# tim-oster/voxel-rs

Measured on AMD Instinct MI355X. Metric: Mrays/sec (primary+shadow) at 1920x1080, depth-12 SVO; achieved HBM GB/s, higher is better.
Workload: dtype f32

## Files before the change

### profiles/timeline.py

```python
#!/usr/bin/env python3
import argparse
import json
import os
import sys
from pathlib import Path

os.environ["VX_TIMELINE"] = "1"
ROOT = Path(__file__).resolve().parent.parent
os.environ.setdefault("VX_LIB_DIR", str(ROOT / "voxel-rs_amd" / "lib" / "lib_tl"))
sys.path.insert(0, str(ROOT))
from _pkg import load_package

vra = load_package()
from voxel_rs_amd import hip, scenes


def main():
    ap = argparse.ArgumentParser()
    ap.add_argument("--format", default="esvo")
    ap.add_argument("--depth", type=int, default=12)
    ap.add_argument("--hot", default="1")
    ap.add_argument("--width", type=int, default=1920)
    ap.add_argument("--height", type=int, default=1080)
    args = ap.parse_args()
# ... 11 lines not shown
    svo.update(world)
    svo.set_frames_in_flight(1)
    u = scenes.bench_camera(args.depth, st["h_max"], W, H, shadow_distance=3.0e38, render_shadows=True)
    image = torch.zeros((H, W, 4), dtype=torch.float32, device="cuda")
    torch.cuda.synchronize()
    svo.profile_enable(True)
    for _ in range(6):
        svo.render_device(u, W, H, image.data_ptr())
    svo.sync()
    ms, launches = svo.profile_read()
    svo.profile_enable(False)
    raw = svo.timeline()
    r6 = raw[:, 6].copy()
    adv_only, push_only = ((r6 >> np.uint64(20)) & np.uint64(0xfffff)).astype(np.float64), ((r6 >> np.uint64(40)) & np.uint64(0xfffff)).astype(np.float64)
    raw[:, 6] = r6 & np.uint64(0xfffff)
    t = raw.astype(np.float64)
    t0 = t[:, 0].min()
    start, empty, leave = (t[:, 0] - t0) / 100.0, (t[:, 1] - t0) / 100.0, (t[:, 2] - t0) / 100.0
    q = lambda a: [round(float(np.percentile(a, p)), 1) for p in (0, 10, 50, 90, 99, 100)]
    r7 = t[:, 7].astype(np.uint64)
    wp, wt, wc = (r7 >> np.uint64(52)).astype(np.float64), ((r7 >> np.uint64(32)) & np.uint64(0xfffff)).astype(np.float64), (r7 & np.uint64(0xffffffff)).astype(np.float64)
    fit = [round(float(v), 1) for v in np.linalg.lstsq(np.stack([wp, wt], axis=1), wc, rcond=None)[0]] if wp.sum() > 0 else None
    print(json.dumps({"format": args.format, "hot_first": args.hot, "waves": int(len(t)), "percentiles": [0, 10, 50, 90, 99, 100],
                      "start_us": q(start), "queue_empty_us": q(empty[t[:, 1] > 0]), "exit_us": q(leave), "tail_us_per_wave": q((leave - empty)[t[:, 1] > 0]),
                      "subtiles_taken": q(t[:, 3].astype(np.uint64) & np.uint64(0xfffff)),
                      "service_phases_per_wave": q((t[:, 3].astype(np.uint64) >> np.uint64(20)) & np.uint64(0xfff)),
                      "us_in_service_phases_per_wave": q((t[:, 3].astype(np.uint64) >> np.uint64(32)).astype(np.float64) / 100.0), "kernel_us": round(float(leave.max()), 1),
                      "kernel_us_by_events_mean_of_launches": round(ms / max(launches, 1) * 1e3, 1),
                      "mean_wave_lifetime_us": round(float((leave - start).mean()), 1),
                      "clock_mhz": q(t[:, 4] / np.maximum(t[:, 2] - t[:, 0], 1.0) * 100.0),
                      "loop_share_of_wave_life": q(t[:, 5] / np.maximum(t[:, 4], 1.0)),
                      "loop_trips_per_wave": q(t[:, 6]),
                      "trips_by_tail_advance_only_push_only_merged": [round(float(adv_only.sum() / max(t[:, 6].sum(), 1.0)), 3), round(float(push_only.sum() / max(t[:, 6].sum(), 1.0)), 3),
                                                                      round(float(1.0 - (adv_only.sum() + push_only.sum()) / max(t[:, 6].sum(), 1.0)), 3)],
                      "cycles_per_trip_as_a_wave_sees_it": q(t[:, 5] / np.maximum(t[:, 6], 1.0)),
                      "cycles_per_trip_mean": round(float(t[:, 5].sum() / max(t[:, 6].sum(), 1.0)), 1),
                      "simd_cycles_per_trip_at_4_waves": round(float(t[:, 5].sum() / max(t[:, 6].sum(), 1.0)) / 4.0, 1),
                      "walk_phases_per_wave": q(wp), "walk_trips_per_wave": q(wt), "walk_cycles_per_wave": q(wc), "walk_fit_cycles_per_phase_and_per_trip": fit}))


if __name__ == "__main__":
    main()
```

### voxel-rs_amd/csrc/hip/comm.cpp

```cpp
#include <dlfcn.h>

#include <cstring>

#include "vx_context.hpp"

using vxrt::fail;
using vxrt::ProfiledLaunch;

namespace {

struct Rccl {
    void* lib = nullptr;
    decltype(&ncclGetUniqueId) GetUniqueId = nullptr;
    decltype(&ncclCommInitRank) CommInitRank = nullptr;
    decltype(&ncclCommDestroy) CommDestroy = nullptr;
    decltype(&ncclGroupStart) GroupStart = nullptr;
    decltype(&ncclGroupEnd) GroupEnd = nullptr;
    decltype(&ncclSend) Send = nullptr;
    decltype(&ncclRecv) Recv = nullptr;
    decltype(&ncclGetErrorString) GetErrorString = nullptr;
};
Rccl g_rccl;
std::string g_rccl_path;

// ... 102 lines not shown
int gather_tiles(vx_context* ctx, const void* tiles, uint64_t bytes_per_rank, void* gathered, int root, int* out_ticket, int only_slot);
}

int vx_gather_tiles(vx_context* ctx, const void* tiles, uint64_t bytes_per_rank, void* gathered, int root, int* out_ticket) {
    return gather_tiles(ctx, tiles, bytes_per_rank, gathered, root, out_ticket, -1);
}

namespace {
int gather_tiles(vx_context* ctx, const void* tiles, uint64_t bytes_per_rank, void* gathered, int root, int* out_ticket, int only_slot) {
    if (!ctx || !tiles || !bytes_per_rank || (bytes_per_rank & 3)) return fail(VX_ERR_INVALID_ARGUMENT, "gather_tiles: bad argument");
    VX_LOCK(ctx);
    if (!ctx->comm) return fail(VX_ERR_STATE, "gather_tiles: no communicator (vx_comm_init)");
    if (root < 0 || root >= ctx->comm_ranks) return fail(VX_ERR_INVALID_ARGUMENT, "gather_tiles: bad root");
    if (ctx->comm_rank == root && !gathered) return fail(VX_ERR_INVALID_ARGUMENT, "gather_tiles: the root needs a destination");
    HIP_TRY(hipSetDevice(ctx->device));
    if (only_slot >= 0 && only_slot < vx_context::kFrameStreams && ctx->frame_recorded[only_slot]) {
        HIP_TRY(hipStreamWaitEvent(ctx->comm_stream, ctx->frame_done[only_slot], 0));
    } else {
        if (ctx->render_recorded) HIP_TRY(hipStreamWaitEvent(ctx->comm_stream, ctx->render_done, 0));
        for (int i = 0; i < vx_context::kFrameStreams; ++i)
            if (ctx->frame_recorded[i]) HIP_TRY(hipStreamWaitEvent(ctx->comm_stream, ctx->frame_done[i], 0));
    }
    const size_t words = size_t(bytes_per_rank / 4);
    ProfiledLaunch ev{};
    if (ctx->profile) {
        if (!ctx->event_pool.empty()) {
            ev = ctx->event_pool.back();
            ctx->event_pool.pop_back();
        } else {
            HIP_TRY(hipEventCreate(&ev.start));
            HIP_TRY(hipEventCreate(&ev.stop));
        }
        HIP_TRY(hipEventRecord(ev.start, ctx->comm_stream));
    }
    auto exchange = [&]() -> int {
        if (ctx->comm_rank == root) {
// ... 95 lines not shown
```

### voxel-rs_amd/csrc/hip/kernels_render.hip

```cpp
#include <hip/hip_runtime.h>

#include "kernels.h"
#include "vx_device.hpp"
#include "vx_loop_gfx950.hpp"

#ifndef VX_ASM_LOOP
#define VX_ASM_LOOP 1
#endif
#ifndef VX_TIMELINE_BUILD
#define VX_TIMELINE_BUILD 0
#endif

using namespace vxd;
using namespace vxk;

namespace {


__device__ __forceinline__ uint32_t xcd_remap(uint32_t b, uint32_t n) {
    constexpr uint32_t X = 8;
    const uint32_t per = n / X, rem = n % X;
    const uint32_t xcd = b % X, slot = b / X;
    const uint32_t start = xcd * per + (xcd < rem ? xcd : rem);
    return start + slot;
// ... 157 lines not shown
    uint32_t out_index = 0;
    float primary_rd[3] = {0, 0, 0};
    float keep_color[4] = {0, 0, 0, 0}, keep_ds = 0.0f;
    float held_t = -1.0f;
    constexpr bool kDescendAlong = IMAGE && !HOT;
    vx_hit rec;
    uint32_t steps = 0;
    Counters ctr = {};
    uint32_t n_pixels = 0, lit = 0, shadow_rays = 0;
    uint32_t wave_steps = 0, services = 0, refills = 0, tail_wave_steps = 0, tail_iterations = 0;

    uint32_t cursor = 64, sub = 0;
    bool queue_empty = false;
    const unsigned long long t_start = a.timeline ? __builtin_amdgcn_s_memrealtime() : 0ull;
    unsigned long long t_empty = 0ull;
    uint32_t taken = 0;
    uint32_t in_service = 0, service_phases = 0;
    const unsigned long long c_start = a.timeline ? __builtin_amdgcn_s_memtime() : 0ull;
    unsigned long long loop_cycles = 0ull;
    uint32_t loop_trips = 0;
    unsigned long long loop_tails = 0ull;
    uint32_t my_queue = blockIdx.x & (kQueues - 1u);
    auto draw_raw = [&]() -> uint32_t {
        uint32_t raw = 0;
        if (lane == 0) raw = atomicAdd(a.work_counter + my_queue * kQueueStride, 1u);
        return raw;
    };
    auto region_ticket = [&](uint32_t k, uint32_t queue) -> uint32_t { return queue_subtile(k, queue, a.stripe, a.stripe_shift); };
    auto ticket_of = [&](uint32_t raw, uint32_t queue) -> uint32_t {
        return region_ticket(((gridDim.x + kQueues - 1u - queue) >> 3) + uint32_t(__builtin_amdgcn_readfirstlane(raw)), queue);
// ... 7 lines not shown
        for (uint32_t tried = 1; t >= a.total_subtiles && tried < kQueues; ++tried) {
            my_queue = (my_queue + 1u) & (kQueues - 1u);
            t = ticket_of(draw_raw(), my_queue);
        }
        return t;
    };
    if (blockIdx.x == 0 && lane < kQueues) a.next_counter[lane * kQueueStride] = 0u;
    uint32_t walk_cycles = 0, walk_trips = 0, walk_phases = 0;
    uint32_t my_chunk = 0, my_fill = 0;

    for (;;) {
        const uint32_t park_limit = a.service_min + uint32_t(__popcll(__ballot(state == kIdle || (FOREIGN == VX_SVO_CSVO && state == kForeign))));
        const uint32_t keep_going = park_limit >= 64u ? 0u : 64u - park_limit;
        unsigned long long trav = __ballot(tr.iter < uint32_t(kMaxSteps));
        const unsigned long long c_loop = a.timeline ? __builtin_amdgcn_s_memtime() : 0ull;
        constexpr bool kAsmLoop = VX_ASM_LOOP != 0 && IMAGE && (LV == kLdsLevels || LV == 16) && !HOT && !STATS;
        bool by_hand = false;
        if constexpr (kAsmLoop) {
            by_hand = __ballot((tr.flags & Trav<SVO>::kHasAdjacentLeaf) != 0 && tr.iter < uint32_t(kMaxSteps)) == 0;
            if (SVO == VX_SVO_IMAGE_WIDE && sc.wide_bytes >= (uint64_t(1) << 35)) by_hand = false;
        }
        if (kAsmLoop && by_hand) {
            if constexpr (kAsmLoop) {
                const uint32_t lds_base = uint32_t(reinterpret_cast<uintptr_t>(fast_st.at(0)));
                const uint32_t lds_slot0 = lds_base + fast_st.slot0;
                const uint32_t lds_aux0 = lds_base + 2u * FastStack::kPlane + uint32_t(int32_t(fast_st.slot0) >> 1);
                const uint32_t f_waiting = FOREIGN == VX_SVO_CSVO ? uint32_t(__popcll(__ballot(state == kForeign))) : 0u;
                const uint32_t f_min = FOREIGN == VX_SVO_CSVO ? 1u : 0xffffffffu;
                constexpr int kForeignKind = FOREIGN == VX_SVO_CSVO ? 1 : (FOREIGN == kForeignRerun ? 2 : 0);
                if (a.timeline) traverse_loop_gfx950<SVO, kForeignKind, true, LV>(tr, sc.records8, sc.wide, lds_slot0, lds_aux0, keep_going, f_waiting, f_min, loop_trips, &loop_tails);
// ... 324 lines not shown
                    }
                }
            }
        }
        VX_PART_END(4);
#undef VX_PART_BEGIN
#undef VX_PART_END
        if (a.timeline) { if (a.timeline_part == 0) in_service += uint32_t(__builtin_amdgcn_s_memrealtime() - t_service); ++service_phases; }
        if (__ballot(state != kIdle) == 0 && queue_empty) break;
    }

    if (a.timeline && lane == 0) {
        unsigned long long* row = a.timeline + size_t(blockIdx.x) * 8;
        row[0] = t_start; row[1] = t_empty; row[2] = __builtin_amdgcn_s_memrealtime();
        row[3] = taken | ((unsigned long long)(service_phases & 0xfffu) << 20) | ((unsigned long long)in_service << 32);
        row[4] = __builtin_amdgcn_s_memtime() - c_start; row[5] = loop_cycles;
        row[6] = (unsigned long long)(loop_trips & 0xfffffu) | ((loop_tails & 0xfffffull) << 20) | (((loop_tails >> 32) & 0xfffffull) << 40);
        row[7] = ((unsigned long long)(walk_phases & 0xfffu) << 52) | ((unsigned long long)(walk_trips & 0xfffffu) << 32) | walk_cycles;
    }
    if (FOREIGN == kForeignRerun || (FOREIGN == VX_SVO_CSVO && !HITS)) {
        const DevScene sc_bytes = vouched(make_scene(sa));
        Stack<64, false, false, int(FullStack::kStackBytes / (64u * 12u))> st2;
        st2.init(lane, &spill);
        const float to_light[3] = {-p.u.light_dir[0], -p.u.light_dir[1], -p.u.light_dir[2]};
        for (uint32_t c = my_chunk; c != 0;) {
            const uint32_t* chunk = todo.chunks + size_t(c - 1) * kRayChunkDwords;
            const uint32_t n = __builtin_amdgcn_readfirstlane(chunk[1]);
            c = __builtin_amdgcn_readfirstlane(chunk[0]);
            if (lane < n) {
                const uint4* w = reinterpret_cast<const uint4*>(chunk + kRayChunkHeader + lane * kRayRecordDwords);
                const uint4 w0 = w[0];
// ... 122 lines not shown
```

### voxel-rs_amd/csrc/hip/runtime.cpp

```cpp
#include <algorithm>
#include <chrono>
#include <cmath>
#include <cstdio>
#include <cstdlib>
#include <cstring>
#include <new>
#include <thread>

#include "vx_context.hpp"

using namespace vxd;
using namespace vxk;
using vxrt::check_ready;
using vxrt::fail;
using vxrt::g_last_error;
using vxrt::kWorldPad;
using vxrt::ProfiledLaunch;

namespace vxrt {
thread_local std::string g_last_error;
int fail(int code, const std::string& msg) {
    g_last_error = msg;
    return code;
}
// ... 9 lines not shown
    s.width = c->tex.width; s.height = c->tex.height; s.layers = c->tex.layers; s.levels = c->tex.levels;
    for (int l = 0; l < 16; ++l) s.level_offset[l] = c->tex.level_offset[l];
    return s;
}

int check_ready(vx_context* ctx) {
    if (!ctx) return fail(VX_ERR_INVALID_ARGUMENT, "null context");
    HIP_TRY(hipSetDevice(ctx->device));
    if (!ctx->committed) return fail(VX_ERR_STATE, "no SVO committed yet (call vx_commit / vx_commit_all first)");
    return VX_OK;
}

int mark_world_read(vx_context* ctx) {
    HIP_TRY(hipEventRecord(ctx->render_done, ctx->stream));
    ctx->render_recorded = true;
    return VX_OK;
}
}


namespace {
void wait_commit_idle(vx_context* ctx);
void stop_commit_worker(vx_context* ctx);
}

namespace {

constexpr size_t kImagePad = 64;
constexpr size_t kStagingSlack = 64;

// ... 217 lines not shown
            hs->width = p.width; hs->height = p.height; hs->tile_rank = p.tile_rank; hs->tile_count = p.tile_count;
        }
        a.stripe = 1;
        if (!a.order) a.stripe = ctx->queue_stripe > 0 ? uint32_t(ctx->queue_stripe) : 16u;
        if (a.stripe > a.total_subtiles) a.stripe = a.total_subtiles;
        if (a.stripe < 1u) a.stripe = 1u;
        a.stripe_shift = 0xffffffffu;
        for (uint32_t b = 0; b < 32u; ++b)
            if (a.stripe == (1u << b)) a.stripe_shift = b;
        int per_cu_used = per_cu;
        if (ctx->waves_per_cu_cap > 0 && ctx->waves_per_cu_cap < per_cu) per_cu_used = ctx->waves_per_cu_cap;
        else if (ctx->comm_ranks > 1 && ctx->comm_headroom > 0 && per_cu > ctx->comm_headroom + 4) per_cu_used = per_cu - ctx->comm_headroom;
        else if (p.tile_count > 1 || ctx->comm) per_cu_used = per_cu > 4 ? per_cu - 1 : per_cu;
        uint32_t waves = uint32_t(ctx->cu_count) * uint32_t(per_cu_used);
        if (waves > a.total_subtiles) waves = a.total_subtiles;
        if (waves > 8192) a.timeline = nullptr;
        ctx->timeline_waves = a.timeline ? waves : 0;
        PixelList todo = {nullptr, nullptr, 0};
        if (imaged && ctx->svo_type == VX_SVO_CSVO) {
            uint32_t*& ring = slot >= 0 ? ctx->d_frame_todo[slot] : ctx->d_main_todo;
            size_t& have = slot >= 0 ? ctx->frame_todo_chunks[slot] : ctx->main_todo_chunks;
            const bool ray_list = !HITS;
            const size_t need = ray_list ? (size_t(p.n_local_tiles) * kTile * kTile / kRayChunkRecords + waves + 1) * (kRayChunkDwords / kChunkDwords)
                                         : size_t(p.n_local_tiles) * kTile * kTile / 63 + waves + 1;
            if (have < need) {
                if (ring) {
                    HIP_TRY(hipStreamSynchronize(stream));
                    (void)hipFree(ring);
                    ring = nullptr;
                    have = 0;
                }
// ... 6 lines not shown
            todo.next_chunk = ring;
            todo.chunks = ring + 32;
            todo.mask = uint32_t((ray_list ? have / (kRayChunkDwords / kChunkDwords) : have) - 1);
        }
        void* kargs[] = {const_cast<SceneArgs*>(&sc), const_cast<RenderParams*>(&p), &a, &out, &hits, &counters, &todo};
        HIP_TRY(hipLaunchKernel(fn, dim3(waves), dim3(64), kargs, wave_lds, stream));
        tickets += 1u;
        order_after = hs;
        order_subtiles = a.total_subtiles;
    }
    HIP_TRY(hipGetLastError());
    if (ctx->profile) {
        HIP_TRY(hipEventRecord(ev.stop, stream));
        ctx->launches.push_back(ev);
    }
    if (slot >= 0) {
        HIP_TRY(hipEventRecord(ctx->frame_done[slot], stream));
        ctx->frame_recorded[slot] = true;
    } else {
        HIP_TRY(hipEventRecord(ctx->render_done, stream));
        ctx->render_recorded = true;
    }
    if (order_after) {
        vx_context::HotState* hs = order_after;
        const uint32_t g = hs->frames % 3;
        {
            HIP_TRY(hipStreamWaitEvent(ctx->order_stream, slot >= 0 ? ctx->frame_done[slot] : ctx->render_done, 0));
            HIP_TRY(vxk::launch_order(ctx->order_stream, hs->cost[g], hs->tag, order_subtiles, hs->order[g]));
            HIP_TRY(hipEventRecord(hs->order_done[g], ctx->order_stream));
        }
        hs->frames += 1;
    }
    ctx->last_frame_slot = slot;
    return VX_OK;
}

int apply_pending_waits(vx_context* ctx, hipStream_t stream) {
    if (ctx->pending_wait) HIP_TRY(hipStreamWaitEvent(stream, ctx->pending_wait, 0));
    if (ctx->pending_gather) HIP_TRY(hipStreamWaitEvent(stream, ctx->pending_gather, 0));
    ctx->pending_wait = nullptr;
    ctx->pending_gather = nullptr;
// ... 223 lines not shown
    {
        if (const char* e = std::getenv("VX_RENDER_KERNEL")) c->kernel_version = std::atoi(e) == 1 ? 1 : 2;
        if (const char* e = std::getenv("VX_FRAMES_IN_FLIGHT")) c->frames_in_flight = std::atoi(e);
        if (c->frames_in_flight < 1) c->frames_in_flight = 1;
        if (c->frames_in_flight > vx_context::kFrameStreams) c->frames_in_flight = vx_context::kFrameStreams;
        if (const char* e = std::getenv("VX_TRAVERSAL_IMAGE")) c->image_enabled = std::atoi(e) != 0;
        if (const char* e = std::getenv("VX_FOREIGN_RERUN")) c->foreign_rerun = std::atoi(e) != 0 ? 1 : 0;
        if (const char* e = std::getenv("VX_HOT_LEVELS")) c->hot_levels = std::atoi(e) != 0;
        if (const char* e = std::getenv("VX_IMAGE_CAP_BYTES")) c->image_cap_bytes = size_t(std::strtoull(e, nullptr, 10));
        if (const char* e = std::getenv("VX_IMAGE_FIRST_BYTES")) c->image_first_bytes = std::max<size_t>(4096, size_t(std::strtoull(e, nullptr, 10)));
        int wide_image = 0;
        if (const char* e = std::getenv("VX_WIDE_IMAGE")) wide_image = std::atoi(e);
        c->image = vximg::WorldImage(svo_type, wide_image ? vximg::kOct64Wide : vximg::kOct64, wide_image == 2 ? (uint64_t(5) << 30) / 4 : 0);
        if (const char* e = std::getenv("VX_COMM_HEADROOM")) c->comm_headroom = std::max(0, std::atoi(e));
        if (const char* e = std::getenv("VX_SERVICE_MIN")) c->service_min = uint32_t(std::atoi(e));
        c->tile_numbering = svo_type == VX_SVO_ESVO ? 2 : 1;
        if (const char* e = std::getenv("VX_TILE_NUMBERING")) c->tile_numbering = std::atoi(e);
        if (vxk::timeline_build()) {
            if (const char* e = std::getenv("VX_HOT_FIRST")) c->hot_first = std::atoi(e) != 0;
            if (const char* e = std::getenv("VX_TIMELINE"))
                if (std::atoi(e) != 0) CREATE_TRY(hipMalloc(reinterpret_cast<void**>(&c->d_timeline), 8192 * 8 * sizeof(unsigned long long)));
            if (const char* e = std::getenv("VX_TIMELINE_PART")) c->timeline_part = uint32_t(std::atoi(e));
            if (const char* e = std::getenv("VX_WAVES_PER_CU")) c->waves_per_cu_cap = std::atoi(e);
            if (const char* e = std::getenv("VX_REFILL_MIN")) c->refill_min = uint32_t(std::atoi(e));
            if (const char* e = std::getenv("VX_QUEUE_STRIPE")) c->queue_stripe = std::atoi(e);
            if (const char* e = std::getenv("VX_TILE_STRIP")) c->tile_strip = std::atoi(e);
        }
        if (c->refill_min < 1) c->refill_min = 1;
        if (c->refill_min > 64) c->refill_min = 64;
        if (c->service_min < 1) c->service_min = 1;
        if (c->service_min > 64) c->service_min = 64;
    }
    const vx_material zero_mat = {0, 0, -1, -1, -1, -1, -1, -1};
    CREATE_TRY(hipMalloc(reinterpret_cast<void**>(&c->d_materials), sizeof zero_mat));
    CREATE_TRY(hipMemcpy(c->d_materials, &zero_mat, sizeof zero_mat, hipMemcpyHostToDevice));
    c->n_materials = 1;
// ... 270 lines not shown
                drop_image();
            }
        }
    } else if (ctx->image_enabled && ctx->kernel_version != 1) {
        drop_image();
    }
    if (image_ok) {
        const uint8_t* src = reinterpret_cast<const uint8_t*>(ctx->image.frame().data());
        if (whole_image) {
            up.push_back(Upload{ctx->d_image, src, ctx->image.frame_bytes()});
        } else {
            for (const vximg::Range& r : ctx->image.dirty_bytes()) up.push_back(Upload{ctx->d_image + r.start, src + r.start, r.length});
        }
    }

    auto wait_for_frames = [&]() -> int {
        if (ctx->render_recorded) HIP_TRY(hipStreamWaitEvent(ctx->upload_stream, ctx->render_done, 0));
        for (int i = 0; i < vx_context::kFrameStreams; ++i)
            if (ctx->frame_recorded[i]) HIP_TRY(hipStreamWaitEvent(ctx->upload_stream, ctx->frame_done[i], 0));
        return VX_OK;
    };
    uint64_t total = 0;
    for (const Upload& u : up) total += u.bytes;
    int rc = VX_OK;
    if (total <= kDeltaLimit) {
        rc = upload_packed(ctx, up, wait_for_frames);
    } else {
        rc = wait_for_frames();
        if (rc == VX_OK) rc = upload_big(ctx, up);
    }
    if (rc != VX_OK) {
        const std::string why = g_last_error;
        drop_image();
        ctx->image_ok = false;
        g_last_error = why;
        return rc;
// ... 178 lines not shown
    if (ps.busy) HIP_TRY(hipEventSynchronize(ps.copied));
    if (ps.cap < bytes) {
        if (ps.dev) (void)hipFree(ps.dev);
        if (ps.host) (void)hipHostFree(ps.host);
        ps.dev = ps.host = nullptr;
        ps.cap = 0;
        HIP_TRY(hipMalloc(&ps.dev, bytes));
        HIP_TRY(hipHostMalloc(&ps.host, bytes, hipHostMallocDefault));
        ps.cap = bytes;
    }
    if (!ps.copied) HIP_TRY(hipEventCreateWithFlags(&ps.copied, hipEventDisableTiming));
    if (!ctx->copy_stream) HIP_TRY(hipStreamCreateWithFlags(&ctx->copy_stream, hipStreamNonBlocking));
    const int slot = ctx->frames_in_flight > 1 ? int(ctx->frame_index++ % unsigned(ctx->frames_in_flight)) : -1;
    if (int rc = apply_pending_waits(ctx, slot >= 0 ? ctx->frame_stream[slot] : ctx->stream)) return rc;
    if (int rc = launch_render(ctx, p, static_cast<float*>(ps.dev), nullptr, nullptr, slot)) return rc;
    HIP_TRY(hipStreamWaitEvent(ctx->copy_stream, slot >= 0 ? ctx->frame_done[slot] : ctx->render_done, 0));
    HIP_TRY(hipMemcpyAsync(ps.host, ps.dev, bytes, hipMemcpyDeviceToHost, ctx->copy_stream));
    HIP_TRY(hipEventRecord(ps.copied, ctx->copy_stream));
    ps.bytes = bytes;
    ps.busy = true;
    *out_slot = k;
    return VX_OK;
}

int vx_present_wait(vx_context* ctx, int slot, const void** pixels, size_t* bytes) {
    if (!ctx || slot < 0 || slot >= vx_context::kPresentSlots || !pixels) return fail(VX_ERR_INVALID_ARGUMENT, "present_wait: bad argument");
    VX_LOCK(ctx);
    vx_context::PresentSlot& ps = ctx->present[slot];
    if (!ps.busy) return fail(VX_ERR_STATE, "present_wait: nothing was begun on this slot");
    HIP_TRY(hipSetDevice(ctx->device));
// ... 122 lines not shown
    return VX_OK;
}

int vx_wait_event(vx_context* ctx, void* hip_event) {
    if (!ctx) return fail(VX_ERR_INVALID_ARGUMENT, "null context");
    VX_LOCK(ctx);
    ctx->pending_wait = static_cast<hipEvent_t>(hip_event);
    return VX_OK;
}

int vx_stream_wait_render(vx_context* ctx, void* stream) {
    if (!ctx) return fail(VX_ERR_INVALID_ARGUMENT, "null context");
    VX_LOCK(ctx);
    HIP_TRY(hipSetDevice(ctx->device));
    const int slot = ctx->last_frame_slot;
    if (slot >= 0) {
        if (ctx->frame_recorded[slot]) HIP_TRY(hipStreamWaitEvent(static_cast<hipStream_t>(stream), ctx->frame_done[slot], 0));
    } else if (ctx->render_recorded) {
        HIP_TRY(hipStreamWaitEvent(static_cast<hipStream_t>(stream), ctx->render_done, 0));
    }
    return VX_OK;
}

int vx_assemble_tiles(vx_context* ctx, const float* tiles, uint64_t stride_floats, uint32_t tile_count, uint32_t width, uint32_t height,
                      float* out_rgba32f) {
    if (!ctx) return fail(VX_ERR_INVALID_ARGUMENT, "null context");
    for (int i = 0; i < vx_context::kFrameStreams; ++i)
        if (ctx->frame_recorded[i]) HIP_TRY(hipStreamWaitEvent(ctx->stream, ctx->frame_done[i], 0));
    return vx_assemble_tiles_on(ctx, tiles, stride_floats, tile_count, width, height, out_rgba32f, ctx->stream);
}

int vx_assemble_tiles_on(vx_context* ctx, const float* tiles, uint64_t stride_floats, uint32_t tile_count, uint32_t width, uint32_t height,
                         float* out_rgba32f, void* stream) {
    if (stride_floats & 3) return fail(VX_ERR_INVALID_ARGUMENT, "assemble_tiles: the stride between the ranks' lists must be whole pixels (a multiple of 4 floats)");
    return vx_assemble_tiles_format(ctx, tiles, stride_floats / 4, tile_count, width, height, out_rgba32f, VX_FORMAT_RGBA32F, stream);
}

int vx_assemble_tiles_format(vx_context* ctx, const void* tiles, uint64_t stride_pixels, uint32_t tile_count, uint32_t width, uint32_t height, void* out,
                             int format, void* stream) {
    if (!ctx || !tiles || !out || !tile_count || !width || !height || (format != VX_FORMAT_RGBA32F && format != VX_FORMAT_RGBA8))
        return fail(VX_ERR_INVALID_ARGUMENT, "assemble_tiles: bad argument");
    const uintptr_t align = format == VX_FORMAT_RGBA32F ? 15u : 3u;
    if ((reinterpret_cast<uintptr_t>(tiles) & align) || (reinterpret_cast<uintptr_t>(out) & align))
// ... 87 lines not shown
        }
        if (!ctx->h_probe) HIP_TRY(hipHostMalloc(reinterpret_cast<void**>(&ctx->h_probe), 2 * sizeof(unsigned long long), hipHostMallocDefault));
        ctx->h_probe[0] = ctx->h_probe[1] = 0ull;
        HIP_TRY(vxk::launch_clock_probe(ctx->probe_stream, microseconds * 100u, ctx->h_probe));
    }
    HIP_TRY(hipStreamSynchronize(ctx->probe_stream));
    if (ctx->h_probe[1] == 0ull) return fail(VX_ERR_HIP, "clock_probe: the probe did not report");
    *shader_mhz = double(ctx->h_probe[0]) / double(ctx->h_probe[1]) * 100.0;
    return VX_OK;
}

uint32_t vx_timeline_read(vx_context* ctx, uint64_t* out, uint32_t capacity_waves) {
    if (!ctx || !ctx->d_timeline || !out) return 0;
    VX_LOCK(ctx);
    if (hipSetDevice(ctx->device) != hipSuccess || drain_streams(ctx) != VX_OK) return 0;
    const uint32_t n = ctx->timeline_waves < capacity_waves ? ctx->timeline_waves : capacity_waves;
    if (n && hipMemcpy(out, ctx->d_timeline, size_t(n) * 8 * sizeof(uint64_t), hipMemcpyDeviceToHost) != hipSuccess) return 0;
    return n;
}

int vx_image_info(const vx_context* ctx, uint64_t out[4]) {
    if (!ctx || !out) return fail(VX_ERR_INVALID_ARGUMENT, "image_info: null argument");
    VX_LOCK(const_cast<vx_context*>(ctx));
    out[0] = ctx->image_ok ? (ctx->pub.layout == vximg::kOct64Wide ? 2u : 1u) : 0u;
    out[1] = ctx->image_ok ? ctx->pub.frame_bytes : 0u;
    out[2] = ctx->image_ok ? ctx->pub.origin_bytes : 0u;
    out[3] = ctx->image_ok ? ctx->pub.chunks : 0u;
    return VX_OK;
}

// ... 28 lines not shown
```

### voxel-rs_amd/csrc/hip/vx_context.hpp

```cpp
#pragma once

#include <hip/hip_runtime_api.h>
#include <rccl/rccl.h>

#include <condition_variable>
#include <mutex>
#include <string>
#include <thread>
#include <unordered_map>
#include <vector>

#include "kernels.h"
#include "traversal_image.hpp"
#include "voxel_hip.h"
#include "vx_args.hpp"

namespace vxrt {

extern thread_local std::string g_last_error;
int fail(int code, const std::string& msg);

#define HIP_TRY(call)                                                                                              \
    do {                                                                                                           \
        hipError_t e_ = (call);                                                                                    \
// ... 3 lines not shown

struct ProfiledLaunch {
    hipEvent_t start, stop;
};

}

struct vx_context;
namespace vxrt {
void comm_release(vx_context* c);

constexpr size_t kWorldPad = 16;
vxd::SceneArgs scene_on_bytes(const vx_context* c);
int check_ready(vx_context* ctx);
int mark_world_read(vx_context* ctx);
}

struct vx_context {
    int svo_type = 0;
    int device = 0;
    size_t capacity = 0;
    uint8_t* staging = nullptr;
    uint8_t* d_world = nullptr;
    hipStream_t stream = nullptr;
    hipStream_t upload_stream = nullptr;
    hipEvent_t upload_done = nullptr, render_done = nullptr;
    bool committed = false, render_recorded = false;
    static constexpr int kFrameStreams = 8;
    hipStream_t frame_stream[kFrameStreams] = {};
    hipEvent_t frame_done[kFrameStreams] = {};
    bool frame_recorded[kFrameStreams] = {};
    uint32_t* d_frame_counter[kFrameStreams] = {};
    uint32_t frame_tickets[kFrameStreams] = {};
    uint32_t* d_frame_todo[kFrameStreams] = {};
    size_t frame_todo_chunks[kFrameStreams] = {};
    uint32_t* d_main_todo = nullptr;
    size_t main_todo_chunks = 0;
    uint32_t main_tickets = 0;
    struct HotState {
        uint32_t* cost[3] = {nullptr, nullptr, nullptr};
        uint32_t* order[3] = {nullptr, nullptr, nullptr};
        hipEvent_t order_done[3] = {nullptr, nullptr, nullptr};
        size_t subtiles = 0;
        uint32_t tag = 0;
        uint32_t frames = 0;
        uint32_t width = 0, height = 0, tile_rank = 0, tile_count = 0;
// ... 17 lines not shown
    float* d_frame = nullptr;  size_t d_frame_bytes = 0;
    vx_hit* d_hits = nullptr;  size_t d_hits_bytes = 0;
    vx_picker_task* d_tasks = nullptr;  vx_picker_result* d_results = nullptr;  uint32_t picker_cap = 0;
    static constexpr uint32_t kPickerDirect = 2048;
    vx_picker_task* h_pick_tasks = nullptr;  vx_picker_result* h_pick_results = nullptr;
    vx_picker_task* d_pick_tasks = nullptr;  vx_picker_result* d_pick_results = nullptr;
    vx_result* d_trace_result = nullptr;  vx_frame* d_trace_frames = nullptr;  uint32_t* d_trace_count = nullptr;  uint32_t trace_cap = 0;
    unsigned long long* d_counters = nullptr;

    uint32_t* d_work_counter = nullptr;
    unsigned long long* d_excursions = nullptr;
    bool count_excursions = false;
    unsigned long long* d_timeline = nullptr;
    uint32_t timeline_waves = 0;
    uint32_t timeline_part = 0;
    vximg::WorldImage image;
    uint8_t* d_image = nullptr;
    size_t d_image_capacity = 0;
    uint8_t* d_origin = nullptr;
    size_t d_origin_capacity = 0;
    size_t image_cap_bytes = 0;
    size_t image_first_bytes = size_t(32) << 20;
    struct DeltaSlot { uint8_t* host = nullptr; uint8_t* dev = nullptr; size_t cap = 0; hipEvent_t done = nullptr; bool used = false; };
    static constexpr int kDeltaSlots = 3;
    DeltaSlot delta[kDeltaSlots];
    unsigned delta_next = 0;
    bool hot_levels = false;
    int foreign_rerun = -1;
    bool big = false;
    bool image_enabled = true;
    bool image_ok = false;
    int kernel_version = 2;
    uint32_t refill_min = 64, service_min = 64;
    int tile_strip = 8;
    int tile_numbering = 1;
    int queue_stripe = 0;
    std::vector<vx_material> host_materials;
    std::vector<uint8_t> opaque_layer;
    uint64_t opaque_blocks = 0;
    int waves_per_cu_cap = 0;
    int comm_headroom = 4;
    int cu_count = 256;
    std::unordered_map<const void*, int> persistent_blocks;

    struct TileTable { uint32_t tiles_x = 0, tiles_y = 0; uint32_t* d_order = nullptr; uint32_t* d_inverse = nullptr; };
    std::vector<TileTable> tile_tables;
    struct LaunchTable { uint32_t tiles_x = 0, tiles_y = 0, rank = 0, count = 0, numbering = 0, strip = 0; uint2* d_table = nullptr; uint32_t* d_number = nullptr; };
    std::vector<LaunchTable> launch_tables;

    ncclComm_t comm = nullptr;
    int comm_ranks = 0, comm_rank = 0;
    hipStream_t comm_stream = nullptr;
    static constexpr int kGatherEvents = 16;
    hipEvent_t gather_done[kGatherEvents] = {};
    unsigned gather_index = 0;
// ... 32 lines not shown
```

Measured before the change: 14000.

## Record render-done events lazily and cap waves for tile-list renders

Render launches now mark frames dirty instead of recording a completion event every launch. The event is recorded only when a consumer (gather, copy, upload, assemble) needs to wait on it, which trims per-frame host API calls. For sharded tile-list renders, the persistent wave count is capped to about three subtiles per wave (at least one wave per CU), so tiny launches carry less wave-launch overhead. Timeline instrumentation also gains multi-launch ring storage and a start-to-first-trip timestamp, plus new profiling scripts.

```diff
diff --git a/profiles/round7/ab_summary.py b/profiles/round7/ab_summary.py
--- /dev/null
+++ b/profiles/round7/ab_summary.py
@@ -0,0 +1,57 @@
+#!/usr/bin/env python3
+import glob
+import json
+import statistics
+import sys
+
+d = sys.argv[1]
+
+
+def lines(arm, mode):
+    out = []
+    for f in sorted(glob.glob(f"{d}/{arm}_{mode}_*.json")):
+        try:
+            out.append(json.loads(open(f).read()))
+        except ValueError:
+            pass
+    return out
+
+
+def fit_a(sm):
+    xs, ys = [1 / 2, 1 / 4, 1 / 8], [sm[n]["share_ms_mean"] for n in ("2", "4", "8")]
+    mx, my = sum(xs) / 3, sum(ys) / 3
+    b = sum((x - mx) * (y - my) for x, y in zip(xs, ys)) / sum((x - mx) ** 2 for x in xs)
+    return my - b * mx
+
+
+FIGURES = [("plain", "ms_per_step (plain run, one block of 50)", lambda j: j["ms_per_step"], True),
+           ("full", "ms_per_step burst (--full, median of 25 blocks)", lambda j: j["burst"]["ms_per_step"], True),
+           ("full", "ms_per_step sustained (--full, 3 s)", lambda j: j["sustained"]["ms_per_step"], True),
+           ("full", "scale_model share_ms_mean N=2", lambda j: j["scale_model"]["2"]["share_ms_mean"], True),
+           ("full", "scale_model share_ms_mean N=4", lambda j: j["scale_model"]["4"]["share_ms_mean"], True),
+           ("full", "scale_model share_ms_mean N=8", lambda j: j["scale_model"]["8"]["share_ms_mean"], True),
+           ("full", "scale_model refitted constant a (ms)", lambda j: fit_a(j["scale_model"]), True),
+           ("full", "scale_model projected_speedup N=8", lambda j: j["scale_model"]["8"]["projected_speedup"], False),
+           ("full", "forced_sharded_vs_plain", lambda j: j["config"]["forced_sharded_vs_plain"], False),
+           ("full", "one_frame_at_a_time_wall_ms", lambda j: j["config"]["one_frame_at_a_time_wall_ms"], True)]
+
+print(f"{'figure':52s} {'arm':6s} {'n':>2s} {'median':>9s} {'min':>9s} {'max':>9s}   verdict (new median against the parent's whole spread)")
+for mode, name, get, lower_is_better in FIGURES:
+    rows = {}
+    for arm in ("parent", "new"):
+        v = [get(j) for j in lines(arm, mode)]
+        v = [x for x in v if x is not None]
+        rows[arm] = v
+    if not rows["parent"] or not rows["new"]:
+        print(f"{name:52s} no data")
+        continue
+    pm, nm = statistics.median(rows["parent"]), statistics.median(rows["new"])
+    lo, hi = min(rows["parent"]), max(rows["parent"])
+    if lo <= nm <= hi:
+        verdict = "inside the parent's spread: no gain claimed"
+    else:
+        better = (nm < lo) if lower_is_better else (nm > hi)
+        verdict = f"{'GAIN' if better else 'LOSS'}: {100.0 * (nm / pm - 1.0):+.1f} % on the medians"
+    for arm in ("parent", "new"):
+        v = rows[arm]
+        print(f"{name:52s} {arm:6s} {len(v):2d} {statistics.median(v):9.4f} {min(v):9.4f} {max(v):9.4f}   {verdict if arm == 'new' else ''}")
diff --git a/profiles/round7/grid_sweep.py b/profiles/round7/grid_sweep.py
--- /dev/null
+++ b/profiles/round7/grid_sweep.py
@@ -0,0 +1,86 @@
+#!/usr/bin/env python3
+import argparse
+import json
+import math
+import os
+import sys
+import time
+from pathlib import Path
+
+ROOT = Path(__file__).resolve().parent.parent.parent
+sys.path.insert(0, str(ROOT))
+from _pkg import load_package
+
+vra = load_package()
+from voxel_rs_amd import hip, scenes
+
+
+def moving(depth, h_max, W, H, i):
+    n = float(1 << depth)
+    a = math.radians(0.25 * i)
+    fwd = (0.6 * math.cos(a) - 0.7 * math.sin(a), -0.35, 0.6 * math.sin(a) + 0.7 * math.cos(a))
+    eye = (0.5 * n + 0.05 * i, h_max + 0.05 * n, 0.5 * n + 0.066 * i)
+    return scenes.render_params_to_uniforms(eye, fwd, (0.0, 1.0, 0.0), math.radians(72.0), W / H, 0.3, (-1.0, -1.0, -1.0), True, 3.0e38)
+
+
+def fit(shares):
+    xs, ys = [1.0 / n for n in shares], list(shares.values())
+    mx, my = sum(xs) / len(xs), sum(ys) / len(ys)
+    b = sum((x - mx) * (y - my) for x, y in zip(xs, ys)) / sum((x - mx) ** 2 for x in xs)
+    return my - b * mx, b
+
+
+def main():
+    ap = argparse.ArgumentParser()
+    ap.add_argument("--factors", default="1,2,3,4,6,8,16,65536")
+    ap.add_argument("--format", default="csvo")
+    ap.add_argument("--rounds", type=int, default=2)
+    args = ap.parse_args()
+    import torch
+
+    depth, W, H = 12, 1920, 1080
+    fmt = vra.SVO_ESVO if args.format == "esvo" else vra.SVO_CSVO
+    world = vra.World(fmt)
+    st = world.build_heightfield(depth)
+    views = [moving(depth, st["h_max"], W, H, i) for i in range(50)]
+    tex, mats = scenes.asset_textures(ROOT / "tests" / "golden" / "textures"), scenes.synthetic_materials()
+
+    def timed(svo, frame, steps=30):
+        for i in range(4):
+            frame(i)
+        svo.sync()
+        blocks = []
+        for _ in range(3):
+            t0 = time.perf_counter()
+            for i in range(steps):
+                frame(i)
+            svo.sync()
+            blocks.append((time.perf_counter() - t0) / steps * 1e3)
+        return sorted(blocks)[1]
+
+    for rnd in range(args.rounds):
+        for factor in [int(f) for f in args.factors.split(",")]:
+            os.environ["VX_LIST_SUBTILES_PER_WAVE"] = str(factor)
+            svo = hip.Svo(fmt, world.size_in_bytes + (16 << 20))
+            svo.set_materials(mats)
+            svo.set_textures(tex, 6)
+            svo.update_full(world)
+            shares = {}
+            for n in (2, 4, 8):
+                frames = min(8, max(3, n))
+                svo.set_frames_in_flight(frames)
+                per = max(hip.local_tile_count(W, H, r, n) for r in range(n))
+                lists = [torch.zeros((per, 32, 32, 4), dtype=torch.uint8, device="cuda") for _ in range(frames)]
+                torch.cuda.synchronize()
+                ms = [timed(svo, lambda i, r=r: svo.render_device(views[i % len(views)], W, H, lists[i % frames].data_ptr(), tile_rank=r, tile_count=n, fmt=hip.VX_FORMAT_RGBA8))
+                      for r in range(n)]
+                shares[n] = sum(ms) / n
+                del lists
+            a, b = fit(shares)
+            print(json.dumps({"round": rnd, "subtiles_per_wave": factor, "share_ms_mean": {str(n): round(v, 4) for n, v in shares.items()},
+                              "fit_a_ms": round(a, 4), "fit_b_ms": round(b, 4)}), flush=True)
+            svo.close()
+
+
+if __name__ == "__main__":
+    main()
diff --git a/profiles/round7/launch_cost.py b/profiles/round7/launch_cost.py
--- /dev/null
+++ b/profiles/round7/launch_cost.py
@@ -0,0 +1,131 @@
+#!/usr/bin/env python3
+import argparse
+import ctypes as C
+import json
+import math
+import os
+import sys
+import time
+from pathlib import Path
+
+ROOT = Path(__file__).resolve().parent.parent.parent
+os.environ["VX_TIMELINE"] = "1"
+os.environ.setdefault("VX_TIMELINE_LAUNCHES", "24")
+os.environ.setdefault("VX_LIB_DIR", str(ROOT / "voxel-rs_amd" / "lib" / "lib_tl"))
+sys.path.insert(0, str(ROOT))
+from _pkg import load_package
+
+vra = load_package()
+from voxel_rs_amd import hip, scenes
+
+
+def moving(depth, h_max, W, H, i):
+    n = float(1 << depth)
+    a = math.radians(0.25 * i)
+    fwd = (0.6 * math.cos(a) - 0.7 * math.sin(a), -0.35, 0.6 * math.sin(a) + 0.7 * math.cos(a))
+    eye = (0.5 * n + 0.05 * i, h_max + 0.05 * n, 0.5 * n + 0.066 * i)
+    return scenes.render_params_to_uniforms(eye, fwd, (0.0, 1.0, 0.0), math.radians(72.0), W / H, 0.3, (-1.0, -1.0, -1.0), True, 3.0e38)
+
+
+def read_rows(svo, launches):
+    import numpy as np
+
+    out = np.zeros((launches * 8192, 8), dtype=np.uint64)
+    n = hip.lib().vx_timeline_read(svo._h, out.ctypes.data_as(C.c_void_p), launches * 8192)
+    return out[:n]
+
+
+def figures(rows, launches, frames, slots):
+    import numpy as np
+
+    waves = len(rows) // launches
+    r = rows[: waves * launches].reshape(launches, waves, 8)
+    start, leave = r[:, :, 0].astype(np.float64) / 100.0, r[:, :, 2].astype(np.float64) / 100.0
+    t0 = start.min()
+    start, leave = start - t0, leave - t0
+    to_first = (r[:, :, 4] >> np.uint64(44)).astype(np.float64) / 100.0
+    k_start, k_end = start.min(axis=1), leave.max(axis=1)
+    gaps = [k_start[i + frames] - k_end[i] for i in range(launches - frames)]
+    period = (k_start[-1] - k_start[frames]) / max(launches - 1 - frames, 1)
+    lo, hi = k_start[frames], k_end[launches - frames - 1]
+    ev = np.concatenate([np.stack([start.ravel(), np.ones(start.size)], 1), np.stack([leave.ravel(), -np.ones(leave.size)], 1)])
+    ev = ev[np.argsort(ev[:, 0], kind="stable")]
+    resident = np.cumsum(ev[:, 1])
+    t = ev[:, 0]
+    dt = np.diff(np.clip(t, lo, hi))
+    below = float(dt[resident[:-1] < slots].sum() / max(hi - lo, 1e-9))
+    mean_res = float((dt * resident[:-1]).sum() / max(hi - lo, 1e-9))
+    p = lambda a, q: round(float(np.percentile(a, q)), 2)
+    per_kernel = [{"launch": i, "first_start_us": round(float(k_start[i]), 2), "median_start_us": p(start[i], 50), "last_start_us": round(float(start[i].max()), 2),
+                   "median_exit_us": p(leave[i], 50), "last_exit_us": round(float(k_end[i]), 2), "first_trip_median_us": p(to_first[i], 50),
+                   "first_trip_p95_us": p(to_first[i], 95)} for i in range(launches)]
+    return {"waves_per_launch": int(waves), "launches": launches, "frames_in_flight": frames, "device_wave_slots": slots,
+            "period_us": round(float(period), 2),
+            "gap_us": {"median": p(gaps, 50), "min": p(gaps, 0), "max": p(gaps, 100), "all": [round(float(g), 2) for g in gaps]},
+            "start_to_first_trip_us": {"median": p(to_first, 50), "p95": p(to_first, 95), "p5": p(to_first, 5)},
+            "first_wave_to_median_wave_start_us": p(np.median(start, axis=1) - k_start, 50),
+            "drain_us_last_exit_minus_median_exit": {"median": p(k_end - np.median(leave, axis=1), 50), "max": p(k_end - np.median(leave, axis=1), 100)},
+            "kernel_span_us": {"median": p(k_end - k_start, 50), "sd": round(float(np.std(k_end - k_start)), 2)},
+            "wave_life_us_median": p(leave - start, 50),
+            "below_full_share": round(below, 4), "mean_resident_waves": round(mean_res, 1), "per_kernel": per_kernel}
+
+
+def main():
+    ap = argparse.ArgumentParser()
+    ap.add_argument("--format", default="csvo")
+    ap.add_argument("--depth", type=int, default=12)
+    ap.add_argument("--width", type=int, default=1920)
+    ap.add_argument("--height", type=int, default=1080)
+    ap.add_argument("--raw-dir", default=None)
+    args = ap.parse_args()
+    import numpy as np
+    import torch
+
+    K = int(os.environ["VX_TIMELINE_LAUNCHES"])
+    fmt = vra.SVO_ESVO if args.format == "esvo" else vra.SVO_CSVO
+    W, H = args.width, args.height
+    world = vra.World(fmt)
+    st = world.build_heightfield(args.depth)
+    svo = hip.Svo(fmt, world.size_in_bytes + (16 << 20))
+    svo.set_materials(scenes.synthetic_materials())
+    svo.set_textures(scenes.asset_textures(ROOT / "tests" / "golden" / "textures"), 6)
+    svo.update(world)
+    views = [moving(args.depth, st["h_max"], W, H, i) for i in range(64)]
+    slots = torch.cuda.get_device_properties(0).multi_processor_count * 16
+    out = {"format": args.format, "depth": args.depth, "size": [W, H], "launches_kept": K, "knobs": svo.knobs()}
+
+    def run(name, frames, frame, host_ms=None):
+        svo.set_frames_in_flight(frames)
+        for i in range(2 * K):
+            frame(i)
+        svo.sync()
+        t0 = time.perf_counter()
+        for i in range(K):
+            frame(i)
+        issue = (time.perf_counter() - t0) / K * 1e3
+        svo.sync()
+        wall = (time.perf_counter() - t0) / K * 1e3
+        rows = read_rows(svo, K)
+        f = figures(rows, K, frames if frames > 1 else 1, slots)
+        f["host_issue_ms_per_frame"], f["wall_ms_per_frame"] = round(issue, 4), round(wall, 4)
+        out[name] = f
+        if args.raw_dir:
+            Path(args.raw_dir).mkdir(parents=True, exist_ok=True)
+            np.save(Path(args.raw_dir) / f"{name}.npy", rows[:, :5])
+        print(name, json.dumps({k: v for k, v in f.items() if k != "per_kernel"}), flush=True)
+
+    images = [torch.zeros((H, W, 4), dtype=torch.float32, device="cuda") for _ in range(2)]
+    torch.cuda.synchronize()
+    run("c3_whole_fif2", 2, lambda i: svo.render_device(views[i % len(views)], W, H, images[i % 2].data_ptr()))
+    run("c3_whole_fif1", 1, lambda i: svo.render_device(views[i % len(views)], W, H, images[0].data_ptr()))
+    n, r = 8, 1
+    per = max(hip.local_tile_count(W, H, k, n) for k in range(n))
+    lists = [torch.zeros((per, 32, 32, 4), dtype=torch.uint8, device="cuda") for _ in range(8)]
+    torch.cuda.synchronize()
+    run("share_n8_fif8", 8, lambda i: svo.render_device(views[i % len(views)], W, H, lists[i % 8].data_ptr(), tile_rank=r, tile_count=n, fmt=hip.VX_FORMAT_RGBA8))
+    svo.close()
+    print(json.dumps(out))
+
+
+if __name__ == "__main__":
+    main()
diff --git a/profiles/timeline.py b/profiles/timeline.py
--- a/profiles/timeline.py
+++ b/profiles/timeline.py
@@ -49,6 +49,8 @@
     r6 = raw[:, 6].copy()
     adv_only, push_only = ((r6 >> np.uint64(20)) & np.uint64(0xfffff)).astype(np.float64), ((r6 >> np.uint64(40)) & np.uint64(0xfffff)).astype(np.float64)
     raw[:, 6] = r6 & np.uint64(0xfffff)
+    to_first = (raw[:, 4] >> np.uint64(44)).astype(np.float64) / 100.0
+    raw[:, 4] = raw[:, 4] & np.uint64((1 << 44) - 1)
     t = raw.astype(np.float64)
     t0 = t[:, 0].min()
     start, empty, leave = (t[:, 0] - t0) / 100.0, (t[:, 1] - t0) / 100.0, (t[:, 2] - t0) / 100.0
@@ -63,6 +65,7 @@
                       "us_in_service_phases_per_wave": q((t[:, 3].astype(np.uint64) >> np.uint64(32)).astype(np.float64) / 100.0), "kernel_us": round(float(leave.max()), 1),
                       "kernel_us_by_events_mean_of_launches": round(ms / max(launches, 1) * 1e3, 1),
                       "mean_wave_lifetime_us": round(float((leave - start).mean()), 1),
+                      "start_to_first_trip_us": q(to_first),
                       "clock_mhz": q(t[:, 4] / np.maximum(t[:, 2] - t[:, 0], 1.0) * 100.0),
                       "loop_share_of_wave_life": q(t[:, 5] / np.maximum(t[:, 4], 1.0)),
                       "loop_trips_per_wave": q(t[:, 6]),
diff --git a/voxel-rs_amd/csrc/hip/comm.cpp b/voxel-rs_amd/csrc/hip/comm.cpp
--- a/voxel-rs_amd/csrc/hip/comm.cpp
+++ b/voxel-rs_amd/csrc/hip/comm.cpp
@@ -140,12 +140,13 @@
     if (root < 0 || root >= ctx->comm_ranks) return fail(VX_ERR_INVALID_ARGUMENT, "gather_tiles: bad root");
     if (ctx->comm_rank == root && !gathered) return fail(VX_ERR_INVALID_ARGUMENT, "gather_tiles: the root needs a destination");
     HIP_TRY(hipSetDevice(ctx->device));
+    if (only_slot >= 0 && only_slot < vx_context::kFrameStreams) {
+        if (int rc = vxrt::renders_recorded(ctx, only_slot)) return rc;
+    }
     if (only_slot >= 0 && only_slot < vx_context::kFrameStreams && ctx->frame_recorded[only_slot]) {
         HIP_TRY(hipStreamWaitEvent(ctx->comm_stream, ctx->frame_done[only_slot], 0));
     } else {
-        if (ctx->render_recorded) HIP_TRY(hipStreamWaitEvent(ctx->comm_stream, ctx->render_done, 0));
-        for (int i = 0; i < vx_context::kFrameStreams; ++i)
-            if (ctx->frame_recorded[i]) HIP_TRY(hipStreamWaitEvent(ctx->comm_stream, ctx->frame_done[i], 0));
+        if (int rc = vxrt::wait_for_renders(ctx, ctx->comm_stream)) return rc;
     }
     const size_t words = size_t(bytes_per_rank / 4);
     ProfiledLaunch ev{};
diff --git a/voxel-rs_amd/csrc/hip/kernels_render.hip b/voxel-rs_amd/csrc/hip/kernels_render.hip
--- a/voxel-rs_amd/csrc/hip/kernels_render.hip
+++ b/voxel-rs_amd/csrc/hip/kernels_render.hip
@@ -195,6 +195,7 @@
     bool queue_empty = false;
     const unsigned long long t_start = a.timeline ? __builtin_amdgcn_s_memrealtime() : 0ull;
     unsigned long long t_empty = 0ull;
+    unsigned long long t_first = 0ull;
     uint32_t taken = 0;
     uint32_t in_service = 0, service_phases = 0;
     const unsigned long long c_start = a.timeline ? __builtin_amdgcn_s_memtime() : 0ull;
@@ -232,6 +233,7 @@
         const uint32_t keep_going = park_limit >= 64u ? 0u : 64u - park_limit;
         unsigned long long trav = __ballot(tr.iter < uint32_t(kMaxSteps));
         const unsigned long long c_loop = a.timeline ? __builtin_amdgcn_s_memtime() : 0ull;
+        if (a.timeline && t_first == 0ull && trav != 0ull) t_first = __builtin_amdgcn_s_memrealtime();
         constexpr bool kAsmLoop = VX_ASM_LOOP != 0 && IMAGE && (LV == kLdsLevels || LV == 16) && !HOT && !STATS;
         bool by_hand = false;
         if constexpr (kAsmLoop) {
@@ -586,7 +588,8 @@
         unsigned long long* row = a.timeline + size_t(blockIdx.x) * 8;
         row[0] = t_start; row[1] = t_empty; row[2] = __builtin_amdgcn_s_memrealtime();
         row[3] = taken | ((unsigned long long)(service_phases & 0xfffu) << 20) | ((unsigned long long)in_service << 32);
-        row[4] = __builtin_amdgcn_s_memtime() - c_start; row[5] = loop_cycles;
+        const unsigned long long to_first = t_first > t_start ? t_first - t_start : 0ull;
+        row[4] = ((__builtin_amdgcn_s_memtime() - c_start) & 0xfffffffffffull) | ((to_first < 0xfffffull ? to_first : 0xfffffull) << 44); row[5] = loop_cycles;
         row[6] = (unsigned long long)(loop_trips & 0xfffffu) | ((loop_tails & 0xfffffull) << 20) | (((loop_tails >> 32) & 0xfffffull) << 40);
         row[7] = ((unsigned long long)(walk_phases & 0xfffu) << 52) | ((unsigned long long)(walk_trips & 0xfffffu) << 32) | walk_cycles;
     }
diff --git a/voxel-rs_amd/csrc/hip/runtime.cpp b/voxel-rs_amd/csrc/hip/runtime.cpp
--- a/voxel-rs_amd/csrc/hip/runtime.cpp
+++ b/voxel-rs_amd/csrc/hip/runtime.cpp
@@ -47,6 +47,30 @@
 int mark_world_read(vx_context* ctx) {
     HIP_TRY(hipEventRecord(ctx->render_done, ctx->stream));
     ctx->render_recorded = true;
+    ctx->render_dirty = false;
+    return VX_OK;
+}
+
+int renders_recorded(vx_context* ctx, int slot) {
+    if ((slot == kMainStream || slot == kEveryStream) && ctx->render_dirty) {
+        HIP_TRY(hipEventRecord(ctx->render_done, ctx->stream));
+        ctx->render_dirty = false;
+        ctx->render_recorded = true;
+    }
+    for (int i = 0; i < vx_context::kFrameStreams; ++i)
+        if ((slot == i || slot == kEveryStream) && ctx->frame_dirty[i]) {
+            HIP_TRY(hipEventRecord(ctx->frame_done[i], ctx->frame_stream[i]));
+            ctx->frame_dirty[i] = false;
+            ctx->frame_recorded[i] = true;
+        }
+    return VX_OK;
+}
+
+int wait_for_renders(vx_context* ctx, hipStream_t waiter) {
+    if (int rc = renders_recorded(ctx, kEveryStream)) return rc;
+    if (ctx->render_recorded) HIP_TRY(hipStreamWaitEvent(waiter, ctx->render_done, 0));
+    for (int i = 0; i < vx_context::kFrameStreams; ++i)
+        if (ctx->frame_recorded[i]) HIP_TRY(hipStreamWaitEvent(waiter, ctx->frame_done[i], 0));
     return VX_OK;
 }
 }
@@ -294,7 +318,15 @@
         else if (p.tile_count > 1 || ctx->comm) per_cu_used = per_cu > 4 ? per_cu - 1 : per_cu;
         uint32_t waves = uint32_t(ctx->cu_count) * uint32_t(per_cu_used);
         if (waves > a.total_subtiles) waves = a.total_subtiles;
-        if (waves > 8192) a.timeline = nullptr;
+        if (p.tile_count > 1 && ctx->list_subtiles_per_wave > 1u) {
+            const uint32_t want = std::max((a.total_subtiles + ctx->list_subtiles_per_wave - 1u) / ctx->list_subtiles_per_wave, uint32_t(ctx->cu_count));
+            if (waves > want) waves = want;
+        }
+        if (waves > vx_context::kTimelineRows) a.timeline = nullptr;
+        if (a.timeline && ctx->timeline_launches > 1) {
+            if (waves != ctx->timeline_waves) ctx->timeline_index = 0;
+            a.timeline += size_t(ctx->timeline_index++ % ctx->timeline_launches) * vx_context::kTimelineRows * 8;
+        }
         ctx->timeline_waves = a.timeline ? waves : 0;
         PixelList todo = {nullptr, nullptr, 0};
         if (imaged && ctx->svo_type == VX_SVO_CSVO) {
@@ -331,17 +363,13 @@
         HIP_TRY(hipEventRecord(ev.stop, stream));
         ctx->launches.push_back(ev);
     }
-    if (slot >= 0) {
-        HIP_TRY(hipEventRecord(ctx->frame_done[slot], stream));
-        ctx->frame_recorded[slot] = true;
-    } else {
-        HIP_TRY(hipEventRecord(ctx->render_done, stream));
-        ctx->render_recorded = true;
-    }
+    if (slot >= 0) ctx->frame_dirty[slot] = true;
+    else ctx->render_dirty = true;
     if (order_after) {
         vx_context::HotState* hs = order_after;
         const uint32_t g = hs->frames % 3;
         {
+            if (int rc = vxrt::renders_recorded(ctx, slot)) return rc;
             HIP_TRY(hipStreamWaitEvent(ctx->order_stream, slot >= 0 ? ctx->frame_done[slot] : ctx->render_done, 0));
             HIP_TRY(vxk::launch_order(ctx->order_stream, hs->cost[g], hs->tag, order_subtiles, hs->order[g]));
             HIP_TRY(hipEventRecord(hs->order_done[g], ctx->order_stream));
@@ -595,12 +623,15 @@
         c->image = vximg::WorldImage(svo_type, wide_image ? vximg::kOct64Wide : vximg::kOct64, wide_image == 2 ? (uint64_t(5) << 30) / 4 : 0);
         if (const char* e = std::getenv("VX_COMM_HEADROOM")) c->comm_headroom = std::max(0, std::atoi(e));
         if (const char* e = std::getenv("VX_SERVICE_MIN")) c->service_min = uint32_t(std::atoi(e));
+        if (const char* e = std::getenv("VX_LIST_SUBTILES_PER_WAVE")) c->list_subtiles_per_wave = uint32_t(std::min(65536, std::max(1, std::atoi(e))));
         c->tile_numbering = svo_type == VX_SVO_ESVO ? 2 : 1;
         if (const char* e = std::getenv("VX_TILE_NUMBERING")) c->tile_numbering = std::atoi(e);
         if (vxk::timeline_build()) {
             if (const char* e = std::getenv("VX_HOT_FIRST")) c->hot_first = std::atoi(e) != 0;
+            if (const char* e = std::getenv("VX_TIMELINE_LAUNCHES")) c->timeline_launches = uint32_t(std::min(64, std::max(1, std::atoi(e))));
             if (const char* e = std::getenv("VX_TIMELINE"))
-                if (std::atoi(e) != 0) CREATE_TRY(hipMalloc(reinterpret_cast<void**>(&c->d_timeline), 8192 * 8 * sizeof(unsigned long long)));
+                if (std::atoi(e) != 0)
+                    CREATE_TRY(hipMalloc(reinterpret_cast<void**>(&c->d_timeline), size_t(c->timeline_launches) * vx_context::kTimelineRows * 8 * sizeof(unsigned long long)));
             if (const char* e = std::getenv("VX_TIMELINE_PART")) c->timeline_part = uint32_t(std::atoi(e));
             if (const char* e = std::getenv("VX_WAVES_PER_CU")) c->waves_per_cu_cap = std::atoi(e);
             if (const char* e = std::getenv("VX_REFILL_MIN")) c->refill_min = uint32_t(std::atoi(e));
@@ -901,12 +932,7 @@
         }
     }
 
-    auto wait_for_frames = [&]() -> int {
-        if (ctx->render_recorded) HIP_TRY(hipStreamWaitEvent(ctx->upload_stream, ctx->render_done, 0));
-        for (int i = 0; i < vx_context::kFrameStreams; ++i)
-            if (ctx->frame_recorded[i]) HIP_TRY(hipStreamWaitEvent(ctx->upload_stream, ctx->frame_done[i], 0));
-        return VX_OK;
-    };
+    auto wait_for_frames = [&]() -> int { return vxrt::wait_for_renders(ctx, ctx->upload_stream); };
     uint64_t total = 0;
     for (const Upload& u : up) total += u.bytes;
     int rc = VX_OK;
@@ -1115,6 +1141,7 @@
     const int slot = ctx->frames_in_flight > 1 ? int(ctx->frame_index++ % unsigned(ctx->frames_in_flight)) : -1;
     if (int rc = apply_pending_waits(ctx, slot >= 0 ? ctx->frame_stream[slot] : ctx->stream)) return rc;
     if (int rc = launch_render(ctx, p, static_cast<float*>(ps.dev), nullptr, nullptr, slot)) return rc;
+    if (int rc = vxrt::renders_recorded(ctx, slot)) return rc;
     HIP_TRY(hipStreamWaitEvent(ctx->copy_stream, slot >= 0 ? ctx->frame_done[slot] : ctx->render_done, 0));
     HIP_TRY(hipMemcpyAsync(ps.host, ps.dev, bytes, hipMemcpyDeviceToHost, ctx->copy_stream));
     HIP_TRY(hipEventRecord(ps.copied, ctx->copy_stream));
@@ -1267,6 +1294,7 @@
     VX_LOCK(ctx);
     HIP_TRY(hipSetDevice(ctx->device));
     const int slot = ctx->last_frame_slot;
+    if (int rc = vxrt::renders_recorded(ctx, slot >= 0 ? slot : vxrt::kMainStream)) return rc;
     if (slot >= 0) {
         if (ctx->frame_recorded[slot]) HIP_TRY(hipStreamWaitEvent(static_cast<hipStream_t>(stream), ctx->frame_done[slot], 0));
     } else if (ctx->render_recorded) {
@@ -1278,8 +1306,14 @@
 int vx_assemble_tiles(vx_context* ctx, const float* tiles, uint64_t stride_floats, uint32_t tile_count, uint32_t width, uint32_t height,
                       float* out_rgba32f) {
     if (!ctx) return fail(VX_ERR_INVALID_ARGUMENT, "null context");
-    for (int i = 0; i < vx_context::kFrameStreams; ++i)
-        if (ctx->frame_recorded[i]) HIP_TRY(hipStreamWaitEvent(ctx->stream, ctx->frame_done[i], 0));
+    {
+        VX_LOCK(ctx);
+        HIP_TRY(hipSetDevice(ctx->device));
+        for (int i = 0; i < vx_context::kFrameStreams; ++i) {
+            if (int rc = vxrt::renders_recorded(ctx, i)) return rc;
+            if (ctx->frame_recorded[i]) HIP_TRY(hipStreamWaitEvent(ctx->stream, ctx->frame_done[i], 0));
+        }
+    }
     return vx_assemble_tiles_on(ctx, tiles, stride_floats, tile_count, width, height, out_rgba32f, ctx->stream);
 }
 
@@ -1397,6 +1431,15 @@
     if (!ctx || !ctx->d_timeline || !out) return 0;
     VX_LOCK(ctx);
     if (hipSetDevice(ctx->device) != hipSuccess || drain_streams(ctx) != VX_OK) return 0;
+    if (ctx->timeline_launches > 1) {
+        const uint32_t w = ctx->timeline_waves, kept = std::min(ctx->timeline_index, ctx->timeline_launches);
+        if (!w || uint64_t(w) * kept > capacity_waves) return 0;
+        for (uint32_t k = 0; k < kept; ++k) {
+            const uint32_t part = (ctx->timeline_index - kept + k) % ctx->timeline_launches;
+            if (hipMemcpy(out + size_t(k) * w * 8, ctx->d_timeline + size_t(part) * vx_context::kTimelineRows * 8, size_t(w) * 8 * sizeof(uint64_t), hipMemcpyDeviceToHost) != hipSuccess) return 0;
+        }
+        return w * kept;
+    }
     const uint32_t n = ctx->timeline_waves < capacity_waves ? ctx->timeline_waves : capacity_waves;
     if (n && hipMemcpy(out, ctx->d_timeline, size_t(n) * 8 * sizeof(uint64_t), hipMemcpyDeviceToHost) != hipSuccess) return 0;
     return n;
diff --git a/voxel-rs_amd/csrc/hip/vx_context.hpp b/voxel-rs_amd/csrc/hip/vx_context.hpp
--- a/voxel-rs_amd/csrc/hip/vx_context.hpp
+++ b/voxel-rs_amd/csrc/hip/vx_context.hpp
@@ -41,6 +41,9 @@
 vxd::SceneArgs scene_on_bytes(const vx_context* c);
 int check_ready(vx_context* ctx);
 int mark_world_read(vx_context* ctx);
+constexpr int kMainStream = -1, kEveryStream = -2;
+int renders_recorded(vx_context* ctx, int slot);
+int wait_for_renders(vx_context* ctx, hipStream_t waiter);
 }
 
 struct vx_context {
@@ -57,6 +60,8 @@
     hipStream_t frame_stream[kFrameStreams] = {};
     hipEvent_t frame_done[kFrameStreams] = {};
     bool frame_recorded[kFrameStreams] = {};
+    bool frame_dirty[kFrameStreams] = {};
+    bool render_dirty = false;
     uint32_t* d_frame_counter[kFrameStreams] = {};
     uint32_t frame_tickets[kFrameStreams] = {};
     uint32_t* d_frame_todo[kFrameStreams] = {};
@@ -104,6 +109,8 @@
     unsigned long long* d_timeline = nullptr;
     uint32_t timeline_waves = 0;
     uint32_t timeline_part = 0;
+    static constexpr uint32_t kTimelineRows = 8192;
+    uint32_t timeline_launches = 1, timeline_index = 0;
     vximg::WorldImage image;
     uint8_t* d_image = nullptr;
     size_t d_image_capacity = 0;
@@ -129,6 +136,7 @@
     std::vector<uint8_t> opaque_layer;
     uint64_t opaque_blocks = 0;
     int waves_per_cu_cap = 0;
+    uint32_t list_subtiles_per_wave = 3;
     int comm_headroom = 4;
     int cu_count = 256;
     std::unordered_map<const void*, int> persistent_blocks;
```

Result: no change. 14000, median of 4 (+0.0%).
